# andreaskoepf/faster-rcnn.torch

Hardware: AMD Instinct MI355X
Metric: images/sec (vgg_small 800x450 fwd+bwd) (higher is better)
Workload: dtype f32 (conv / Linear(13824,1024) operands as 2 x fp16 split planes: 22 significand bits, 3 MFMA partial products; fp32 accumulate)

## Files before the change

### faster-rcnn.torch_amd/_lib.py

```python
import ctypes as C
import os

_HERE = os.path.dirname(os.path.abspath(__file__))
SO_PATH = os.environ.get("FRCNN_LIB_PATH") or os.path.join(_HERE, "libfrcnn_hip.so")

KC_NAMES = ["conv_igemm_k3", "conv_igemm_other", "conv_wgrad_k3", "conv_wgrad_other", "gemm", "elemwise",
            "roi", "rpn", "nms", "optim", "image", "conv_x3", "conv_wgradx", "soft_nms", "topk"]


class FrcnnError(RuntimeError):
    pass


class ModelDesc(C.Structure):
    _fields_ = [
        ("nblocks", C.c_int),
        ("filters", C.c_int * 8), ("ksize", C.c_int * 8), ("pad", C.c_int * 8), ("conv_steps", C.c_int * 8),
        ("dropout", C.c_float * 8),
        ("nheads", C.c_int),
        ("head_k", C.c_int * 8), ("head_n", C.c_int * 8), ("head_input", C.c_int * 8),
        ("ncls", C.c_int),
        ("cls_n", C.c_int * 8), ("cls_bn", C.c_int * 8),
        ("cls_dropout", C.c_float * 8),
        ("class_count", C.c_int),
# ... 31 lines not shown
    "frcnn_nms_device_batch": ([vp, C.c_int, C.c_longlong, C.c_int, vp, C.c_int, C.c_float, C.c_int, C.c_int, vp, vp, vp, vp, C.c_size_t,
                               vp], C.c_int),
    "frcnn_soft_nms_workspace_bytes": ([C.c_int, C.c_int], C.c_size_t),
    "frcnn_soft_nms_batch": ([vp, C.c_int, C.c_longlong, C.c_int, vp, C.c_int, C.c_int, C.c_int, C.c_float, C.c_float, C.c_float, C.c_int,
                             vp, vp, vp, vp, C.c_longlong, vp, C.c_size_t, vp], C.c_int),
    "frcnn_topk_select_workspace_bytes": ([C.c_int, C.c_int], C.c_size_t),
    "frcnn_topk_select": ([vp, C.c_int, C.c_longlong, C.c_int, vp, C.c_int, vp, C.c_longlong, vp, vp, C.c_size_t, vp], C.c_int),
    "frcnn_rpn_gather_rows": ([vp, vp, vp, vp, C.c_int, C.c_longlong, C.c_int, vp, C.c_longlong, vp, C.c_int, vp, vp, vp, vp, vp, vp,
                              C.c_longlong, vp], C.c_int),
    "frcnn_detect_gather_batch": ([vp, vp, C.c_int, C.c_int, vp, vp, vp, vp, vp, C.c_longlong, vp, vp, vp, vp, vp], C.c_int),
    "frcnn_roi_windows": ([vp, vp, C.c_int, vp, C.c_int, C.c_int, C.c_int, vp, vp], C.c_int),
    "frcnn_detect_post": ([vp, vp, vp, vp, vp, C.c_int, C.c_int, C.c_double, vp, vp, vp, vp, vp, vp], C.c_int),
    "frcnn_nms_host": ([vp, C.c_int, C.c_int, C.c_float, C.c_int, C.c_int, vp, vp], C.c_int),
    "frcnn_conv2d_forward": ([vp, C.c_int, C.c_int, C.c_int, vp, vp, vp, vp, C.c_int, C.c_int, C.c_int, vp, vp], C.c_int),
    "frcnn_conv2d_backward_input": ([vp, C.c_int, C.c_int, C.c_int, vp, C.c_int, C.c_int, C.c_int, vp, C.c_int, vp], C.c_int),
    "frcnn_conv2d_backward_weight": ([vp, C.c_int, C.c_int, C.c_int, vp, vp, vp, C.c_int, C.c_int, C.c_int, vp, vp, vp], C.c_int),
    "frcnn_maxpool_act_forward": ([vp, C.c_int, C.c_int, C.c_int, vp, vp, vp, vp, vp], C.c_int),
    "frcnn_maxpool_act_backward": ([vp, vp, vp, C.c_int, C.c_int, C.c_int, vp, vp, vp, vp, vp, vp], C.c_int),
    "frcnn_act_forward": ([vp, C.c_int, C.c_longlong, vp, vp, vp, vp], C.c_int),
    "frcnn_act_backward": ([vp, vp, C.c_int, C.c_longlong, vp, vp, vp, vp, vp, vp], C.c_int),
    "frcnn_amax_record_floats": ([], C.c_int),
    "frcnn_tensor_absmax": ([vp, C.c_longlong, vp, vp], C.c_int),
    "frcnn_maxpool_act_forward_rec": ([vp, C.c_int, C.c_int, C.c_int, vp, vp, vp, vp, vp, vp], C.c_int),
    "frcnn_maxpool_act_backward_rec": ([vp, vp, vp, C.c_int, C.c_int, C.c_int, vp, vp, vp, vp, vp, vp, vp], C.c_int),
    "frcnn_act_backward_rec": ([vp, vp, C.c_int, C.c_longlong, vp, vp, vp, vp, vp, vp, vp], C.c_int),
    "frcnn_conv2d_forward_rec": ([vp, C.c_int, C.c_int, C.c_int, vp, vp, vp, vp, C.c_int, C.c_int, C.c_int, vp, vp, vp, vp], C.c_int),
    "frcnn_conv2d_backward_input_rec": ([vp, C.c_int, C.c_int, C.c_int, vp, C.c_int, C.c_int, C.c_int, vp, C.c_int, vp, vp, vp, vp, vp, vp,
                                         vp], C.c_int),
    "frcnn_roi_pool_forward": ([vp, C.c_int, C.c_int, C.c_int, vp, C.c_int, C.c_int, C.c_int, vp, vp, vp], C.c_int),
    "frcnn_roi_pool_backward": ([vp, C.c_int, C.c_int, C.c_int, vp, vp, C.c_int, C.c_int, C.c_int, vp], C.c_int),
# ... 125 lines not shown
```

### faster-rcnn.torch_amd/csrc/api.cpp

```cpp
#include <cmath>
#include <cstring>
#include <vector>
#include <mutex>

#include "kernels.h"

namespace frcnn {

static thread_local std::string g_err;

void set_error(const char* fmt, ...) {
  char buf[1024];
  va_list ap;
  va_start(ap, fmt);
  vsnprintf(buf, sizeof(buf), fmt, ap);
  va_end(ap);
  g_err = buf;
}

struct ProfRec { int klass; double flops, bytes; hipEvent_t a, b; hipStream_t s; };
static hipEvent_t g_prof_base = nullptr;
static unsigned g_prof_mask = 0;
static std::vector<ProfRec> g_recs;
static std::vector<hipEvent_t> g_pool;
// ... 206 lines not shown
  return FRCNN_OK;
}

static int scale_fits_f16_form(const float* in_scale, int C, hipStream_t s, bool* ok) {
  *ok = true;
  if (!in_scale) return FRCNN_OK;
  std::vector<float> h((size_t)C);
  FR_HIP(hipMemcpyAsync(h.data(), in_scale, (size_t)C * 4, hipMemcpyDeviceToHost, s));
  FR_HIP(hipStreamSynchronize(s));
  for (float v : h) if (!(std::fabs(v) <= 1.f)) { *ok = false; break; }
  return FRCNN_OK;
}

static int conv2d_split(const float* in, int Kc, int H, int W, const float* in_slope, const float* in_scale, const float* weight,
                        const float* bias, int O, int C, int M, int k, int mode, int pad, float* out, int out_mode, bool f16,
                        const float* rec_in, float* rec_out, const X3PostAct* post, hipStream_t s) {
  float* wp = nullptr;
  FR_HIP(hipMalloc((void**)&wp, conv_x3_pack_bytes(Kc, M, k)));
  float* am = nullptr;
  int rcx = f16 ? x3_f16_records(&am) : FRCNN_OK;
  float* const amw = am ? am + AMAX_REC : nullptr;
  float* const aws = am ? am + 2 * AMAX_REC : nullptr;
  if (am && rcx == FRCNN_OK) {
    if (!rec_in) rcx = tensor_absmax(in, (long)Kc * H * W, am, s);
    if (rcx == FRCNN_OK) rcx = tensor_absmax(weight, (long)O * C * k * k, amw, s);
  }
  if (rcx == FRCNN_OK) rcx = conv_x3_pack(weight, O, C, k, mode, wp, s, H + 2 * pad - k + 1, W + 2 * pad - k + 1, amw, aws);
  if (rcx == FRCNN_OK)
    rcx = conv_x3(in, Kc, H, W, in_slope, in_scale, wp, bias, M, k, pad, out, out_mode, 0, s, 0, post, am ? (rec_in ? rec_in : am) : nullptr,
                  aws, rec_out);
  (void)hipStreamSynchronize(s);
  (void)hipFree(wp); (void)hipFree(am);
  return rcx;
}

int frcnn_conv2d_forward(const float* in, int C, int H, int W, const float* in_slope, const float* in_scale,
                         const float* weight, const float* bias, int O, int k, int pad, float* out,
                         void* stream) {
  float* wf = nullptr;
  if (conv_x3_eligible(C, O, k) && (k == 3 || (!in_slope && !in_scale))) {
    bool unit = true;
    FR_TRY(scale_fits_f16_form(in_scale, C, S(stream), &unit));
    return conv2d_split(in, C, H, W, in_slope, in_scale, weight, bias, O, C, O, k, 0, pad, out, OUT_STORE, unit, nullptr, nullptr, nullptr,
                        S(stream));
  }
// ... 6 lines not shown
}
int frcnn_conv2d_backward_input(const float* gout, int O, int Ho, int Wo, const float* weight, int C, int k,
                                int pad, float* gin, int accumulate, void* stream) {
  float* wd = nullptr;
  if (conv_x3_eligible(O, C, k))
    return conv2d_split(gout, O, Ho, Wo, nullptr, nullptr, weight, nullptr, O, C, C, k, 1, k - 1 - pad, gin, accumulate ? OUT_ADD : OUT_STORE,
                        true, nullptr, nullptr, nullptr, S(stream));
  FR_HIP(hipMalloc((void**)&wd, conv_pack_floats(O, C, k) * 4));
  int rc = conv_pack_weights(weight, O, C, k, nullptr, wd, S(stream));
  if (rc == FRCNN_OK)
    rc = conv_igemm(gout, O, Ho, Wo, nullptr, nullptr, wd, nullptr, C, k, k - 1 - pad, gin,
                    accumulate ? OUT_ADD : OUT_STORE, 0, S(stream));
  (void)hipStreamSynchronize(S(stream));
  (void)hipFree(wd);
  return rc;
}
int frcnn_amax_record_floats(void) { return AMAX_REC; }
int frcnn_tensor_absmax(const float* x, long long n, float* rec, void* stream) {
  FR_CHECK(x && rec && n >= 1, "frcnn_tensor_absmax: bad arguments");
  return tensor_absmax(x, (long)n, rec, S(stream));
}
int frcnn_conv2d_forward_rec(const float* in, int C, int H, int W, const float* in_slope, const float* in_scale, const float* weight,
                             const float* bias, int O, int k, int pad, float* out, const float* rec_in, float* rec_out, void* stream) {
  FR_CHECK(in && weight && out, "frcnn_conv2d_forward_rec: NULL argument");
  FR_CHECK(conv_x3_eligible(C, O, k) && (k == 3 || (!in_slope && !in_scale)),
           "frcnn_conv2d_forward_rec: %d channels -> %d filters, %dx%d does not take the split form", C, O, k, k);
  FR_CHECK(get_x3_f16(), "frcnn_conv2d_forward_rec: option x3_f16 is off");
  bool unit = true;
  FR_TRY(scale_fits_f16_form(in_scale, C, S(stream), &unit));
  FR_CHECK(unit, "frcnn_conv2d_forward_rec: an entry of in_scale exceeds 1: the launch would not take the fp16 form");
// ... 315 lines not shown
```

### faster-rcnn.torch_amd/csrc/convx.hip

```cpp
#include <cstdlib>

#include "kernels.h"
#include "amax.h"
#include <type_traits>
#ifdef CX_TRACE
#include <cstdio>
#include <vector>
#endif

namespace frcnn {

typedef float f32x16 __attribute__((ext_vector_type(16)));
typedef __bf16 bf16x8 __attribute__((ext_vector_type(8)));
typedef __bf16 bf16x2 __attribute__((ext_vector_type(2)));
typedef float f32x2 __attribute__((ext_vector_type(2)));
typedef _Float16 f16x8 __attribute__((ext_vector_type(8)));
typedef _Float16 f16x2 __attribute__((ext_vector_type(2)));

#define CX_BM 128
#define CX_CH 16
#define CX_OCC 3
#define CX_PP 204
constexpr int cx_pp(int k) { return k == 3 ? CX_PP : k == 5 ? 240 : 308; }
#define CX_NA 2
// ... 9 lines not shown
#define CX_ASTAGE (6 * CX_BM * 16)

static int g_splitbf16 = -1;
void set_split_bf16(int on) { g_splitbf16 = on ? 1 : 0; }
int get_split_bf16() {
  if (g_splitbf16 < 0) g_splitbf16 = getenv("FRCNN_SPLIT_BF16") ? (atoi(getenv("FRCNN_SPLIT_BF16")) != 0) : 1;
  return g_splitbf16;
}

static int g_x3_f16 = -1;
void set_x3_f16(int on) { g_x3_f16 = on ? 1 : 0; }
int get_x3_f16() {
  if (g_x3_f16 < 0) g_x3_f16 = getenv("FRCNN_X3_F16") ? (atoi(getenv("FRCNN_X3_F16")) != 0) : 1;
  return g_x3_f16;
}

bool conv_x3_eligible(int Cin, int M, int k) {
  return get_split_bf16() && (k == 3 || k == 5 || k == 7) && Cin % CX_CH == 0 && Cin >= CX_CH && M % (k == 3 ? 64 : 128) == 0;
}

static void x3_choose_tile(int Ho, int Wo, int k, int* TH, int* TW);
int conv_x3_bm(int M, int Ho, int Wo, int k) {
  if (M % 128 != 0) return 64;
  if (k != 3 || Ho <= 0) return 128;
  int TH, TW;
  x3_choose_tile(Ho, Wo, k, &TH, &TW);
  const long tiles = (long)cdiv(Ho, TH) * cdiv(Wo, TW);
  const long b128 = tiles * (M / 128), b64 = tiles * (M / 64);
  return (b128 < 512 && b64 >= 512 && b64 <= 256 * CX_OCC) ? 64 : 128;
}
// ... 925 lines not shown
    if (FILE* f = fopen(tfile, "w")) {
      fprintf(f, "# grid %d M %d Cin %d Ho %d Wo %d TH %d TW %d splitK %d wide %d WM %d EPI %d\n", grid, a.M, a.Cin, a.Ho, a.Wo, a.TH, a.TW, a.splitK, a.wide, WM, EPI);
      for (int b = 0; b < grid; ++b) {
        for (int j = 0; j < 64; ++j) fprintf(f, "%llu ", hst[(size_t)b * 64 + j]);
        fprintf(f, "\n");
      }
      fclose(f);
    }
  }
#endif
  return FRCNN_OK;
}

int conv_x3(const float* in, int Cin, int H, int W, const float* in_slope, const float* in_scale, const void* wp,
            const float* bias, int M, int k, int pad, float* out, int out_mode, double algo_flops, hipStream_t s, int ws_slot,
            const X3PostAct* post, const float* amax_in, const float* amax_w, float* amax_out) {
  FR_CHECK((k == 3 || k == 5 || k == 7) && Cin % CX_CH == 0 && M % 64 == 0,
           "conv_x3: %d channels -> %d filters, %dx%d is not a split-bf16 shape", Cin, M, k, k);
  FR_CHECK((double)Cin * H * W * 4.0 < 4294967295.0, "conv_x3: input tensor too large for 32-bit offsets");
  CxArgs a;
  a.in = in; a.in_slope = in_slope; a.in_scale = in_scale; a.wp = wp; a.bias = bias; a.out = out;
  a.amax_in = amax_in; a.amax_w = amax_w; a.amax_out = amax_out;
  const bool f16 = amax_in != nullptr;
  FR_CHECK(!f16 || amax_w, "conv_x3: the two-plane fp16 form needs the magnitudes of both tensors");
  a.Cin = Cin; a.H = H; a.W = W; a.M = M; a.pad = pad;
  a.Ho = H + 2 * pad - k + 1; a.Wo = W + 2 * pad - k + 1;
  FR_CHECK(a.Ho > 0 && a.Wo > 0, "conv_x3: empty output (%dx%d, k=%d, pad=%d)", H, W, k, pad);
  x3_choose_tile(a.Ho, a.Wo, k, &a.TH, &a.TW);
  a.tilesX = cdiv(a.Wo, a.TW); a.tilesY = cdiv(a.Ho, a.TH);
  const int bm = conv_x3_bm(M, a.Ho, a.Wo, k);
  a.mTiles = M / bm;
// ... 36 lines not shown
  } else if (post && a.splitK == 1) {
    rc = bm == 128 ? launch_x3<3, 2, false, false, 1>(a, algo_flops, s) : launch_x3<3, 1, false, false, 1>(a, algo_flops, s);
  } else if (k == 3 && bm == 128) {
    rc = act == 3 ? launch_x3<3, 2, true, true>(a, algo_flops, s) : act == 2 ? launch_x3<3, 2, true, false>(a, algo_flops, s)
       : act == 1 ? launch_x3<3, 2, false, true>(a, algo_flops, s) : launch_x3<3, 2, false, false>(a, algo_flops, s);
  } else if (k == 3) {
    rc = act == 3 ? launch_x3<3, 1, true, true>(a, algo_flops, s) : act == 2 ? launch_x3<3, 1, true, false>(a, algo_flops, s)
       : act == 1 ? launch_x3<3, 1, false, true>(a, algo_flops, s) : launch_x3<3, 1, false, false>(a, algo_flops, s);
  } else {
    FR_CHECK(act == 0 && bm == 128, "conv_x3: a %dx%d launch takes no fused input activation and 128-filter blocks", k, k);
    rc = k == 5 ? launch_x3<5, 2, false, false>(a, algo_flops, s) : launch_x3<7, 2, false, false>(a, algo_flops, s);
  }
  FR_TRY(rc);
  if (amax_out && !slab && (long)a.tilesX * a.tilesY * a.mTiles > AMAX_MAX_BLOCKS)
    FR_TRY(tensor_absmax(out, (long)M * a.Ho * a.Wo, amax_out, s));
  if (slab) {
    long total = (long)M * a.Ho * a.Wo;
    int grid;
    const long hw = (long)a.Ho * a.Wo;
    const X3PostAct pa = post ? *post : X3PostAct{nullptr, nullptr, nullptr, nullptr};
    const bool al = ((uintptr_t)out & 15) == 0 && ((uintptr_t)a.out & 15) == 0 && (!post || ((uintptr_t)post->x & 15) == 0);
    const int vec = al && hw % 4 == 0 ? 4 : al && hw % 2 == 0 ? 2 : 1;
    grid = (int)std::min<long>(cdivl(total / vec, 256), 4096);
    if (vec == 4)
      FR_LAUNCH(KC_ELEMWISE, 0, total * 4.0 * (a.splitK + 1), s, x3_splitk_reduce_kernel<4>, dim3(grid), dim3(256), 0,
                (const float*)a.out, a.splitK, M, hw, bias, out, out_mode == OUT_ADD ? 1 : 0, pa, amax_out);
    else if (vec == 2)
      FR_LAUNCH(KC_ELEMWISE, 0, total * 4.0 * (a.splitK + 1), s, x3_splitk_reduce_kernel<2>, dim3(grid), dim3(256), 0,
                (const float*)a.out, a.splitK, M, hw, bias, out, out_mode == OUT_ADD ? 1 : 0, pa, amax_out);
    else
// ... 9 lines not shown
```

### faster-rcnn.torch_amd/csrc/elem.hip

```cpp
#include <algorithm>

#include <mutex>
#include <unordered_map>

#include "kernels.h"
#include "amax.h"

namespace frcnn {

__device__ __forceinline__ float wave_sum(float v) {
#pragma unroll
  for (int o = 32; o > 0; o >>= 1) v += __shfl_down(v, o, 64);
  return v;
}

__device__ __forceinline__ float block_sum(float v, float* sh) {
  v = wave_sum(v);
  const int lane = threadIdx.x & 63, w = threadIdx.x >> 6;
  if (lane == 0) sh[w] = v;
  __syncthreads();
  float r = 0.f;
  if (threadIdx.x < 64) {
    r = threadIdx.x < (blockDim.x >> 6) ? sh[threadIdx.x] : 0.f;
    r = wave_sum(r);
// ... 129 lines not shown
}
int maxpool_act_forward(const float* x, int C, int H, int W, const float* slope, const float* scale,
                        float* out, unsigned char* idx, hipStream_t s, float* amax) {
  int Ho = (H - 2 + 1) / 2 + 1, Wo = (W - 2 + 1) / 2 + 1;
  long total = (long)C * Ho * Wo;
  int grid = (int)std::min<long>(std::max<long>(1, cdivl(total, 256)), 4096);
  FR_LAUNCH(KC_ELEMWISE, 0, (double)C * H * W * 4.0 + total * 5.0, s, maxpool_act_forward_kernel, dim3(grid),
            dim3(256), 0, x, C, H, W, Ho, Wo, slope, scale, out, idx, amax);
  FR_LAUNCH_CHECK();
  return FRCNN_OK;
}

#ifndef ACT_BWD_THREADS
#define ACT_BWD_THREADS 512
#endif
template <bool POOLED, bool VEC>
__global__ __launch_bounds__(ACT_BWD_THREADS) void act_backward_kernel(const float* __restrict__ gin, const unsigned char* __restrict__ idx,
                                    const float* __restrict__ x, int C, int H, int W, int Ho, int Wo,
                                    const float* slope, const float* scale, float* __restrict__ gx,
                                    float* gbias, float* gslope, int chunks, float* part_b, float* part_a, float* amax) {
  __shared__ float sh[16];
  __shared__ double shd[16];
  float am = 0.f;
  const int c = blockIdx.x / chunks, chunk = blockIdx.x % chunks;
  const long hw = (long)H * W;
  long per = cdivl(hw, chunks);
  if (VEC) per = (per + 3) & ~3L;
  const long beg = chunk * per, end = beg + per < hw ? beg + per : hw;
  const float a = slope ? *slope : 1.f;
  const float sc = scale ? scale[c] : 1.f;
  const bool has_slope = slope != nullptr;
  float sb = 0.f;
  double sa = 0.0;
  if (VEC) {
    const float* xc = x + (size_t)c * hw;
    const float* gc = POOLED ? gin + (size_t)c * Ho * Wo : gin + (size_t)c * hw;
    const unsigned char* ic = POOLED ? idx + (size_t)c * Ho * Wo : nullptr;
    float* oc = gx + (size_t)c * hw;
    const unsigned ibeg = (unsigned)beg, iend = (unsigned)end, uW = (unsigned)W, stride = 4u * blockDim.x;
    auto fetch = [&](unsigned i, bool ok, float* g, float4& xv4) {
      if (!ok) { g[0] = g[1] = g[2] = g[3] = 0.f; xv4 = make_float4(1.f, 1.f, 1.f, 1.f); return; }
      if (POOLED) {
        const unsigned y = i / uW, xx = i - y * uW;
        const unsigned po = (y >> 1) * (unsigned)Wo + (xx >> 1);
        const float2 gp = *reinterpret_cast<const float2*>(gc + po);
        const unsigned short ib = *reinterpret_cast<const unsigned short*>(ic + po);
        const unsigned char code = (unsigned char)((y & 1) * 2);
        g[0] = ((ib & 0xff) == code) ? gp.x : 0.f;
        g[1] = ((ib & 0xff) == code + 1) ? gp.x : 0.f;
        g[2] = ((ib >> 8) == code) ? gp.y : 0.f;
        g[3] = ((ib >> 8) == code + 1) ? gp.y : 0.f;
      } else {
        const float4 gv = *reinterpret_cast<const float4*>(gc + i);
        g[0] = gv.x; g[1] = gv.y; g[2] = gv.z; g[3] = gv.w;
      }
      xv4 = *reinterpret_cast<const float4*>(xc + i);
    };
    auto finish = [&](unsigned i, const float* g, const float4& xv4) {
      const float xv[4] = {xv4.x, xv4.y, xv4.z, xv4.w};
      float r[4];
// ... 13 lines not shown
      const bool ok2 = i2 < iend;
      float g0[4], g1[4];
      float4 x0, x1;
      fetch(i, true, g0, x0);
      fetch(i2, ok2, g1, x1);
      finish(i, g0, x0);
      if (ok2) finish(i2, g1, x1);
    }
  } else {
    for (long i = beg + threadIdx.x; i < end; i += blockDim.x) {
      float g;
      if (POOLED) {
        int y = (int)(i / W), xx = (int)(i - (long)y * W);
        int oy = y >> 1, ox = xx >> 1;
        long po = ((long)c * Ho + oy) * Wo + ox;
        g = (idx[po] == (unsigned char)((y & 1) * 2 + (xx & 1))) ? gin[po] : 0.f;
      } else {
        g = gin[(size_t)c * hw + i];
      }
      if (scale) g *= sc;
      float xv = x[(size_t)c * hw + i];
      float r = g;
      if (has_slope) {
        if (!(xv > 0.f)) { r = a * g; sa += (double)xv * (double)g; }
      }
      gx[(size_t)c * hw + i] = r;
      sb += r;
      am = fmaxf(am, fabsf(r));
    }
  }
  if (amax) amax_store_block(am, amax);
// ... 49 lines not shown
    FR_HIP(hipMalloc((void**)&e.first, n * 4));
    e.second = n;
  }
  *out = e.first;
  return FRCNN_OK;
}

static int act_bwd_chunks(int C, long hw) {
  long want = cdivl(512, C);
  long maxc = cdivl(hw, 4096);
  return (int)std::max<long>(1, std::min<long>(want, maxc));
}

int maxpool_act_backward(const float* gpool, const unsigned char* idx, const float* x, int C, int H,
                         int W, const float* slope, const float* scale, float* gx, float* gbias,
                         float* gslope, hipStream_t s, float* amax) {
  int Ho = (H - 2 + 1) / 2 + 1, Wo = (W - 2 + 1) / 2 + 1;
  int chunks = act_bwd_chunks(C, (long)H * W);
  float* const amax_after = (amax && (long)C * chunks > AMAX_MAX_BLOCKS) ? amax : nullptr;
  if (amax_after) amax = nullptr;
  float *pb = nullptr, *pa = nullptr;
  if (deterministic()) { FR_TRY(det_workspace(s, (size_t)2 * C * chunks, &pb)); pa = pb + (size_t)C * chunks; }
  const bool vec = (W % 4 == 0) && (Wo % 2 == 0) && (((uintptr_t)gpool | (uintptr_t)x | (uintptr_t)gx) % 16 == 0) &&
                   ((uintptr_t)idx % 2 == 0);
  if (vec)
    FR_LAUNCH(KC_ELEMWISE, 0, (double)C * H * W * 9.25, s, (act_backward_kernel<true, true>), dim3(C * chunks),
              dim3(ACT_BWD_THREADS), 0, gpool, idx, x, C, H, W, Ho, Wo, slope, scale, gx, gbias, gslope, chunks, pb, pa, amax);
  else
    FR_LAUNCH(KC_ELEMWISE, 0, (double)C * H * W * 9.25, s, (act_backward_kernel<true, false>), dim3(C * chunks),
              dim3(ACT_BWD_THREADS), 0, gpool, idx, x, C, H, W, Ho, Wo, slope, scale, gx, gbias, gslope, chunks, pb, pa, amax);
  FR_LAUNCH_CHECK();
  if (pb) FR_TRY(fold_partials(gbias ? pb : nullptr, (slope && gslope) ? pa : nullptr, C, chunks, gbias, gslope, s));
  if (amax_after) FR_TRY(tensor_absmax(gx, (long)C * H * W, amax_after, s));
  return FRCNN_OK;
}

int act_backward(const float* gy, const float* x, int C, long hw, const float* slope,
                 const float* scale, float* gx, float* gbias, float* gslope, hipStream_t s, float* amax) {
  int chunks = act_bwd_chunks(C, hw);
  float* const amax_after = (amax && (long)C * chunks > AMAX_MAX_BLOCKS) ? amax : nullptr;
  if (amax_after) amax = nullptr;
  float *pb = nullptr, *pa = nullptr;
  if (deterministic()) { FR_TRY(det_workspace(s, (size_t)2 * C * chunks, &pb)); pa = pb + (size_t)C * chunks; }
  const bool vec = (hw % 4 == 0) && (((uintptr_t)gy | (uintptr_t)x | (uintptr_t)gx) % 16 == 0);
  if (vec)
    FR_LAUNCH(KC_ELEMWISE, 0, (double)C * hw * 12.0, s, (act_backward_kernel<false, true>), dim3(C * chunks),
              dim3(ACT_BWD_THREADS), 0, gy, (const unsigned char*)nullptr, x, C, 1, (int)hw, 1, 1, slope, scale, gx,
              gbias, gslope, chunks, pb, pa, amax);
  else
    FR_LAUNCH(KC_ELEMWISE, 0, (double)C * hw * 12.0, s, (act_backward_kernel<false, false>), dim3(C * chunks),
              dim3(ACT_BWD_THREADS), 0, gy, (const unsigned char*)nullptr, x, C, 1, (int)hw, 1, 1, slope, scale, gx,
              gbias, gslope, chunks, pb, pa, amax);
  FR_LAUNCH_CHECK();
  if (pb) FR_TRY(fold_partials(gbias ? pb : nullptr, (slope && gslope) ? pa : nullptr, C, chunks, gbias, gslope, s));
  if (amax_after) FR_TRY(tensor_absmax(gx, (long)C * hw, amax_after, s));
  return FRCNN_OK;
}

__global__ void channel_sum_kernel(const float* __restrict__ g, long hw, float* gbias, int chunks, float* part_b) {
  __shared__ float sh[16];
  const int c = blockIdx.x / chunks, chunk = blockIdx.x % chunks;
  long per = cdivl(hw, chunks);
  per = (per + 3) & ~3L;
  const long beg = chunk * per, end = beg + per < hw ? beg + per : hw;
  const float* gc = g + (size_t)c * hw;
  float sb = 0.f;
  if (beg < end) {
// ... 588 lines not shown
```

### faster-rcnn.torch_amd/csrc/kernels.h

```cpp
#pragma once
#include <algorithm>

#include "common.h"

namespace frcnn {

int conv_cc(int k);
int conv_mpad(int M);
size_t conv_pack_floats(int Kchan, int M, int k);
int conv_pack_weights(const float* w, int O, int C, int k, float* wf, float* wd, hipStream_t s);
struct PackJob { long w_off; long total; float* dst; int O, C, k, mode, Mpad, blk_begin, nblk; };
PackJob conv_pack_job(long w_off, int O, int C, int k, int mode, float* dst);
int conv_pack_assign_blocks(PackJob* jobs, int njobs, int total_blocks);
int conv_pack_weights_multi(const float* weights, const PackJob* jobs_dev, int njobs, int grid, hipStream_t s);

enum { OUT_STORE = 0, OUT_ADD = 1 };
struct IgemmPool { float* out; unsigned char* idx; const float* slope; const float* scale; float* amax = nullptr; };
int conv_igemm(const float* in, int Cin, int H, int W, const float* in_slope, const float* in_scale,
               const float* wp, const float* bias, int M, int k, int pad, float* out, int out_mode,
               double algo_flops, hipStream_t s, int ws_slot = 0,
               const IgemmPool* pool = nullptr, bool* pool_fused = nullptr);

void set_split_bf16(int on);
int get_split_bf16();
// ... 5 lines not shown
};
PackXJob conv_x3_pack_job(long w_off, int O, int C, int k, int mode, void* dst, int Ho, int Wo);
int conv_x3_pack_assign_blocks(PackXJob* jobs, int njobs);
int conv_x3_pack_multi(const float* weights, const PackXJob* jobs_dev, int njobs, int grid, hipStream_t s);
int conv_x3_pack(const float* w, int O, int C, int k, int mode, void* dst, hipStream_t s, int Ho, int Wo,
                 const float* amax_rec_w = nullptr, float* amax_w = nullptr);
#define AMAX_REC 16400
#define AMAX_MAX_BLOCKS 16384
int tensor_absmax(const float* x, long n, float* rec, hipStream_t s);
struct AmaxJob { long off; long n; float* out; int blk_begin; };
int tensor_absmax_assign_blocks(AmaxJob* jobs, int njobs);
long tensor_absmax_record_floats(long n);
int tensor_absmax_multi(const float* w, const AmaxJob* jobs_dev, int njobs, int grid, hipStream_t s);
void set_x3_f16(int on);
int get_x3_f16();
int conv_x3(const float* in, int Cin, int H, int W, const float* in_slope, const float* in_scale, const void* wp,
            const float* bias, int M, int k, int pad, float* out, int out_mode, double algo_flops, hipStream_t s, int ws_slot = 0,
            const struct X3PostAct* post = nullptr, const float* amax_in = nullptr, const float* amax_w = nullptr,
            float* amax_out = nullptr);
struct X3PostAct {
  const float* x;
  const float* slope;
  const float* scale;
  float* gslope;
};

bool conv_wgradx_eligible(int Cin, int O, int k);
size_t conv_wgradx_workspace_bytes(int Cin, int H, int W, int O, int pad);
struct WgradMap { const int* omap = nullptr; const int* cmap = nullptr; int Cfull = 0; };
int conv_wgradx(const float* in, int Cin, int H, int W, const float* in_slope, const float* in_scale, const float* g, int O,
                int pad, float* gw, void* ws, size_t ws_bytes, hipStream_t s, float* gbias = nullptr,
                const float* amax_in = nullptr, const float* amax_g = nullptr,
                const WgradMap* map = nullptr);
int wgrad_reduce(const float* slab, int nSplit, int taps, int OC, float* gw, hipStream_t s);
// ... 11 lines not shown
               const WgradMap* map = nullptr);

bool deterministic();
void set_deterministic(bool on);
int det_workspace(hipStream_t s, size_t floats, float** out);

int fill_zero(void* p, size_t bytes, hipStream_t s);
int scale_inplace(float* x, long n, float sc, hipStream_t s);
int add_inplace(float* y, const float* x, long n, hipStream_t s);
int act_forward(const float* x, int C, long hw, const float* slope, const float* scale, float* y,
                hipStream_t s);
int maxpool_act_forward(const float* x, int C, int H, int W, const float* slope, const float* scale,
                        float* out, unsigned char* idx, hipStream_t s, float* amax = nullptr);
int maxpool_act_backward(const float* gpool, const unsigned char* idx, const float* x, int C, int H,
                         int W, const float* slope, const float* scale, float* gx, float* gbias,
                         float* gslope, hipStream_t s, float* amax = nullptr);
int act_backward(const float* gy, const float* x, int C, long hw, const float* slope,
                 const float* scale, float* gx, float* gbias, float* gslope, hipStream_t s, float* amax = nullptr);
int channel_sum(const float* g, int C, long hw, float* gbias, hipStream_t s);
int channel_sum_cols(const float* g, int R, int O, float* gb, hipStream_t s);
int gather_positions(const float* src, int C, long hw, const int* pos, int P, float* dst, const float* slope,
                     float* dst_act, hipStream_t s);
int im2col_positions(const float* X, int C, int H, int W, int k, int Wo, const int* pos, int P, float* col, hipStream_t s);
int col2im_positions_add(const float* col, int C, int H, int W, int k, int Wo, const int* pos, int P, float* gX,
                         hipStream_t s);
int dropout_channel_mask(float* scale, int C, float p, unsigned long long seed, hipStream_t s);
int fill_value(float* x, long n, float v, hipStream_t s);
int rmsprop_step(float* x, float* g, float* m, long n, float lr, float alpha, float eps, float gscale,
                 bool scale_first, hipStream_t s, const double* gcount_dev = nullptr);
int rmsprop_slice(float* x, float* g, float* m, long lo, long hi, float lr, float alpha, float eps, float gscale, bool scale_first,
                  hipStream_t s, const double* gcount_dev = nullptr);
// ... 173 lines not shown
```

### faster-rcnn.torch_amd/csrc/net.cpp

```cpp
#include <array>
#include <vector>
#include <cmath>
#include <cstring>

#include "kernels.h"

namespace frcnn {

static const int HEAD_OUT = 18;
static const int SPARSE_MAX_POS = 512;

struct DevBuf {
  void* p = nullptr;
  size_t bytes = 0;
  bool owned = true;
  void view(void* ptr, size_t n) { p = ptr; bytes = n; owned = false; }
  int ensure(size_t need) {
    if (need <= bytes) return FRCNN_OK;
    if (p && owned) (void)hipFree(p);
    owned = true;
    p = nullptr; bytes = 0;
    FR_HIP(hipMalloc(&p, need + 64));
    bytes = need;
    return FRCNN_OK;
// ... 664 lines not shown
  return FRCNN_OK;
}

int frcnn_get_option(const char* name, int* value) {
  FR_CHECK(name != nullptr && value != nullptr, "get_option: null argument");
  if (strcmp(name, "side_stream") == 0) { *value = side_enabled() ? 1 : 0; return FRCNN_OK; }
  if (strcmp(name, "gemm_x_roles") == 0) { *value = get_gemm_x_roles(); return FRCNN_OK; }
  if (strcmp(name, "deterministic") == 0) { *value = deterministic() ? 1 : 0; return FRCNN_OK; }
  if (strcmp(name, "static_weights") == 0) { *value = g_static_weights; return FRCNN_OK; }
  if (strcmp(name, "drop_compact") == 0) { *value = drop_compact_on(); return FRCNN_OK; }
  if (strcmp(name, "sparse_heads") == 0) { *value = sparse_heads_on(); return FRCNN_OK; }
  if (strcmp(name, "winograd") == 0) { *value = 0; return FRCNN_OK; }
  if (strcmp(name, "cnet_wgrad_async") == 0) { *value = g_cnet_wgrad_async; return FRCNN_OK; }
  if (strcmp(name, "split_bf16") == 0) { *value = get_split_bf16(); return FRCNN_OK; }
  if (strcmp(name, "x3_f16") == 0) { *value = get_x3_f16(); return FRCNN_OK; }
  FR_CHECK(false, "get_option: unknown option '%s'", name);
  return FRCNN_OK;
}

int frcnn_set_option(const char* name, int value) {
  FR_CHECK(name != nullptr, "set_option: null name");
  if (strcmp(name, "side_stream") == 0) { g_side_stream = value ? 1 : 0; return FRCNN_OK; }
  if (strcmp(name, "deterministic") == 0) { set_deterministic(value != 0); return FRCNN_OK; }
  if (strcmp(name, "static_weights") == 0) { g_static_weights = value != 0; ++g_static_gen; return FRCNN_OK; }
  if (strcmp(name, "drop_compact") == 0) { g_drop_compact = value != 0; return FRCNN_OK; }
  if (strcmp(name, "sparse_heads") == 0) { g_sparse_heads = value != 0; return FRCNN_OK; }
  if (strcmp(name, "gemm_x_roles") == 0) { set_gemm_x_roles(value); return FRCNN_OK; }
  if (strcmp(name, "split_bf16") == 0) { set_split_bf16(value); return FRCNN_OK; }
  if (strcmp(name, "x3_f16") == 0) { set_x3_f16(value); return FRCNN_OK; }
  if (strcmp(name, "winograd") == 0) return FRCNN_OK;
  if (strcmp(name, "cnet_wgrad_async") == 0) { g_cnet_wgrad_async = value ? 1 : 0; return FRCNN_OK; }
  FR_CHECK(false, "set_option: unknown option '%s'", name);
  return FRCNN_OK;
}

static int ensure_head_streams(frcnn_model* m);
static int ensure_side(frcnn_model* m) {
  if (!m->side) {
    FR_TRY(pool_stream(0, &m->side));
    FR_HIP(hipEventCreateWithFlags(&m->join_ev, hipEventDisableTiming));
    FR_HIP(hipEventCreateWithFlags(&m->loss_ev, hipEventDisableTiming));
    FR_HIP(hipEventCreateWithFlags(&m->chain_ev, hipEventDisableTiming));
    for (auto& h : m->heads) FR_HIP(hipEventCreateWithFlags(&h.done, hipEventDisableTiming));
  }
// ... 845 lines not shown
  for (int b = 0; b < fb; ++b) {
    while (m->block_ev.size() < (size_t)nb) {
      hipEvent_t e;
      FR_HIP(hipEventCreateWithFlags(&e, hipEventDisableTiming));
      m->block_ev.push_back(e);
    }
    FR_HIP(hipEventRecord(m->block_ev[b], s));
    FR_TRY(record_block_read(m, b, s));
  }
  const bool use_side = side_enabled();
  if (use_side) FR_TRY(ensure_side(m));
  hipStream_t ws = use_side ? m->side : s;
  size_t n_fork = 0;
  const bool fuse_act = !deterministic() && !(getenv("FRCNN_FUSE_ACT") && atoi(getenv("FRCNN_FUSE_ACT")) == 0);
  bool act_done = false;
  for (int b = nb - 1; b >= fb; --b) {
    Block& blk = m->blocks[b];
    for (int st = blk.nconv - 1; st >= 0; --st) {
      Conv& c = m->convs[blk.first_conv + st];
      const float* scale = (st == 0 && blk.has_drop) ? blk.scale.f() : nullptr;
      const bool fused_here = act_done;
      act_done = false;
      static const bool first_pooled_on = !(getenv("FRCNN_FIRST_POOLED") && atoi(getenv("FRCNN_FIRST_POOLED")) == 0);
      const bool first_pooled = fuse_act && first_pooled_on && b == 0 && st == 0 && blk.nconv == 1 && scale == nullptr &&
                                conv_wgrad_first_pooled_eligible(c.Cin, c.Cout, c.k, c.Wo);
      if (first_pooled) {
        FR_TRY(conv_wgrad_first_pooled(m->img.f(), c.Cin, c.H, c.W, blk.gpooled.f(), (const unsigned char*)blk.pidx.p, c.x.f(),
                                       w + c.a_off, c.Cout, c.pad, grad + c.w_off, grad + c.b_off, grad + c.a_off,
                                       m->wg_ws_first.p, m->wg_ws_first.bytes, s));
        while (m->block_ev.size() < (size_t)nb) {
          hipEvent_t e;
          FR_HIP(hipEventCreateWithFlags(&e, hipEventDisableTiming));
          m->block_ev.push_back(e);
        }
        FR_HIP(hipEventRecord(m->block_ev[b], s));
        FR_TRY(record_block_read(m, b, s));
        break;
      }
      if (fused_here) {
      } else if (st == blk.nconv - 1) {
        FR_TRY(maxpool_act_backward(blk.gpooled.f(), (const unsigned char*)blk.pidx.p, c.x.f(), c.Cout, c.Ho, c.Wo,
                                    w + c.a_off, scale, c.gx.f(), grad + c.b_off, grad + c.a_off, s,
                                    (c.x_d && m->f16_packed) ? m->rec_w(c.am + 1) : nullptr));
      } else {
        FR_TRY(act_backward(c.gx.f(), c.x.f(), c.Cout, (long)c.Ho * c.Wo, w + c.a_off, scale, c.gx.f(),
                            grad + c.b_off, grad + c.a_off, s, (c.x_d && m->f16_packed) ? m->rec_w(c.am + 1) : nullptr));
      }
      const float* in; const float* in_slope = nullptr; const float* in_scale = nullptr;
      if (st > 0) {
        Conv& pc = m->convs[blk.first_conv + st - 1];
        in = pc.x.f(); in_slope = w + pc.a_off;
        in_scale = (st - 1 == 0 && blk.has_drop) ? blk.scale.f() : nullptr;
      } else {
        in = b == 0 ? m->img.f() : m->blocks[b - 1].pooled.f();
      }
      const bool dc = blk.dc_on && st <= 1;
      int wg_cin = c.Cin, wg_o = c.Cout;
      WgradMap wmap;
// ... 31 lines not shown
        break;
      }
      float* gin = st > 0 ? m->convs[blk.first_conv + st - 1].gx.f() : m->blocks[b - 1].gpooled.f();
      const int gmode = st > 0 ? OUT_STORE : OUT_ADD;
      const float* ag = nullptr;
      const float* aw = nullptr;
      if (c.x_d && m->f16_packed) { ag = m->rec(c.am + 1); aw = m->amax_ws.f() + c.am; }
      const int dg_k = (dc && st == 0) ? blk.nkK : c.Cout, dg_m = (dc && st == 1) ? blk.nkM : c.Cin;
      const double fl = 2.0 * dg_k * dg_m * c.k * c.k * (double)c.Ho * c.Wo;
      if (c.x_d && st > 0 && fuse_act && c.k == 3) {
        Conv& pc = m->convs[blk.first_conv + st - 1];
        X3PostAct post{pc.x.f(), w + pc.a_off, (st - 1 == 0 && blk.has_drop && !dc) ? blk.scale.f() : nullptr, grad + pc.a_off};
        FR_TRY(conv_x3(c.gx.f(), dg_k, c.Ho, c.Wo, nullptr, nullptr, c.wxd.p, nullptr, dg_m, c.k, c.k - 1 - c.pad, gin, gmode, fl, s, 0, &post, ag, aw,
                       (pc.x_d && m->f16_packed) ? m->rec_w(pc.am + 1) : nullptr));
        act_done = true;
      } else if (c.x_d)
        FR_TRY(conv_x3(c.gx.f(), dg_k, c.Ho, c.Wo, nullptr, nullptr, c.wxd.p, nullptr, dg_m, c.k, c.k - 1 - c.pad, gin, gmode, fl, s, 0, nullptr, ag, aw));
      else
        FR_TRY(conv_igemm(c.gx.f(), c.Cout, c.Ho, c.Wo, nullptr, nullptr, c.wd.f(), nullptr, c.Cin, c.k,
                          c.k - 1 - c.pad, gin, gmode, fl, s));
      if (st == 0) FR_TRY(record_block_read(m, b, s));
    }
  }
  m->block_ev_valid = true;
  if (heads_tail && !m->heads_gin) FR_TRY(join_heads(m, s));
  FR_TRY(cw_join(m, s));
  if (use_side) {
    FR_HIP(hipEventRecord(m->join_ev, ws));
    FR_HIP(hipStreamWaitEvent(s, m->join_ev, 0));
    m->side_busy = false;
  }
  return FRCNN_OK;
}
// ... 242 lines not shown
```

### include/frcnn_hip.h

```cpp
#ifndef FRCNN_HIP_H
#define FRCNN_HIP_H

#include <stddef.h>

#ifdef __cplusplus
extern "C" {
#endif

#define FRCNN_OK 0
#define FRCNN_ERR_ARG 1
#define FRCNN_ERR_HIP 2
#define FRCNN_ERR_STATE 3

int frcnn_version(void);
const char *frcnn_last_error(void);
int frcnn_device_count(int *n);
int frcnn_set_device(int device);
int frcnn_device_name(char *buf_host, int len);
int frcnn_set_option(const char *name, int value);
int frcnn_get_option(const char *name, int *value_host);

int frcnn_malloc(void **ptr_out_host, size_t bytes);
int frcnn_free(void *ptr);
int frcnn_host_alloc(void **ptr_out_host, size_t bytes);
// ... 47 lines not shown
int frcnn_roi_windows(const double *rect, const long long *pick, int k, const int *layers_host, int nlayers, int fmH, int fmW,
                      int *wins, void *stream);
int frcnn_detect_post(const int *cls, const float *conf, const float *bbox, const double *rect, const long long *pick, int R,
                      int bgclass, double min_conf, float *bb, int *kc, int *keep_row, double *r2, int *K_dev, void *stream);
int frcnn_detect_gather_batch(const long long *wpick, const int *counts, int B, int row_stride, const int *keep_row,
                              const int *kc, const float *bb, const double *r2, const long long *pick, long long match_stride,
                              const float *match_p, const double *match_rect, const int *match_idx, double *rec, void *stream);
int frcnn_nms_host(const float *boxes_host, int n, int ncols, float overlap, int key_mode,
                   int key_col, long long *pick_host, int *count_host);

int frcnn_conv2d_forward(const float *in, int C, int H, int W, const float *in_slope,
                         const float *in_scale, const float *weight, const float *bias, int O,
                         int k, int pad, float *out, void *stream);
int frcnn_conv2d_backward_input(const float *gout, int O, int Ho, int Wo, const float *weight,
                                int C, int k, int pad, float *gin, int accumulate, void *stream);
int frcnn_conv2d_backward_weight(const float *in, int C, int H, int W, const float *in_slope,
                                 const float *in_scale, const float *gout, int O, int k, int pad,
                                 float *gweight, float *gbias, void *stream);

int frcnn_maxpool_act_forward(const float *x, int C, int H, int W, const float *slope,
                              const float *scale, float *out, unsigned char *idx, void *stream);
int frcnn_maxpool_act_backward(const float *gpool, const unsigned char *idx, const float *x, int C,
                               int H, int W, const float *slope, const float *scale, float *gx,
                               float *gbias, float *gslope, void *stream);
int frcnn_act_forward(const float *x, int C, long long hw, const float *slope, const float *scale,
                      float *y, void *stream);
int frcnn_act_backward(const float *gy, const float *x, int C, long long hw, const float *slope,
                       const float *scale, float *gx, float *gbias, float *gslope, void *stream);

int frcnn_amax_record_floats(void);
// ... 200 lines not shown
```

Measured before the change: 518.7.

## Defer split-K slab reduction of dgrad conv into pooled activation backward

When the split-K backward-input convolution writes into the previous block's pooled gradient, the slab reduction is skipped and handed to the following maxpool/activation backward kernel. That kernel then sums the split-K partial slabs (plus the existing value in add mode) inline, removing one reduction pass and one write and read of the pooled gradient. A new API entry and an option toggle are added. The risk is extra strided slab reads inside the elementwise kernel and reliance on the slab staying valid until the consumer runs.

```diff
diff --git a/faster-rcnn.torch_amd/_lib.py b/faster-rcnn.torch_amd/_lib.py
--- a/faster-rcnn.torch_amd/_lib.py
+++ b/faster-rcnn.torch_amd/_lib.py
@@ -69,6 +69,8 @@
     "frcnn_nms_host": ([vp, C.c_int, C.c_int, C.c_float, C.c_int, C.c_int, vp, vp], C.c_int),
     "frcnn_conv2d_forward": ([vp, C.c_int, C.c_int, C.c_int, vp, vp, vp, vp, C.c_int, C.c_int, C.c_int, vp, vp], C.c_int),
     "frcnn_conv2d_backward_input": ([vp, C.c_int, C.c_int, C.c_int, vp, C.c_int, C.c_int, C.c_int, vp, C.c_int, vp], C.c_int),
+    "frcnn_conv2d_backward_input_pool": ([vp, C.c_int, C.c_int, C.c_int, vp, C.c_int, C.c_int, C.c_int, vp, C.c_int, vp, vp, C.c_int, C.c_int,
+                                          vp, vp, vp, vp, vp, vp, vp], C.c_int),
     "frcnn_conv2d_backward_weight": ([vp, C.c_int, C.c_int, C.c_int, vp, vp, vp, C.c_int, C.c_int, C.c_int, vp, vp, vp], C.c_int),
     "frcnn_maxpool_act_forward": ([vp, C.c_int, C.c_int, C.c_int, vp, vp, vp, vp, vp], C.c_int),
     "frcnn_maxpool_act_backward": ([vp, vp, vp, C.c_int, C.c_int, C.c_int, vp, vp, vp, vp, vp, vp], C.c_int),
diff --git a/faster-rcnn.torch_amd/csrc/api.cpp b/faster-rcnn.torch_amd/csrc/api.cpp
--- a/faster-rcnn.torch_amd/csrc/api.cpp
+++ b/faster-rcnn.torch_amd/csrc/api.cpp
@@ -244,7 +244,7 @@
 
 static int conv2d_split(const float* in, int Kc, int H, int W, const float* in_slope, const float* in_scale, const float* weight,
                         const float* bias, int O, int C, int M, int k, int mode, int pad, float* out, int out_mode, bool f16,
-                        const float* rec_in, float* rec_out, const X3PostAct* post, hipStream_t s) {
+                        const float* rec_in, float* rec_out, const X3PostAct* post, hipStream_t s, X3Fold* defer = nullptr) {
   float* wp = nullptr;
   FR_HIP(hipMalloc((void**)&wp, conv_x3_pack_bytes(Kc, M, k)));
   float* am = nullptr;
@@ -258,7 +258,7 @@
   if (rcx == FRCNN_OK) rcx = conv_x3_pack(weight, O, C, k, mode, wp, s, H + 2 * pad - k + 1, W + 2 * pad - k + 1, amw, aws);
   if (rcx == FRCNN_OK)
     rcx = conv_x3(in, Kc, H, W, in_slope, in_scale, wp, bias, M, k, pad, out, out_mode, 0, s, 0, post, am ? (rec_in ? rec_in : am) : nullptr,
-                  aws, rec_out);
+                  aws, rec_out, defer);
   (void)hipStreamSynchronize(s);
   (void)hipFree(wp); (void)hipFree(am);
   return rcx;
@@ -295,6 +295,21 @@
   (void)hipStreamSynchronize(S(stream));
   (void)hipFree(wd);
   return rc;
+}
+int frcnn_conv2d_backward_input_pool(const float* gout, int O, int Ho, int Wo, const float* weight, int C, int k, int pad, float* gin,
+                                     int accumulate, const unsigned char* idx, const float* x, int xH, int xW, const float* slope,
+                                     const float* scale, float* gx, float* gbias, float* gslope, float* rec, void* stream) {
+  FR_CHECK(gout && weight && gin && idx && x && gx, "frcnn_conv2d_backward_input_pool: NULL argument");
+  const int Hi = Ho + k - 1 - 2 * pad, Wi = Wo + k - 1 - 2 * pad;
+  FR_CHECK(xH >= 1 && xW >= 1 && (xH - 1) / 2 + 1 == Hi && (xW - 1) / 2 + 1 == Wi,
+           "frcnn_conv2d_backward_input_pool: x of %d x %d does not pool to the %d x %d map the convolution reads", xH, xW, Hi, Wi);
+  X3Fold fold;
+  if (conv_x3_eligible(O, C, k))
+    FR_TRY(conv2d_split(gout, O, Ho, Wo, nullptr, nullptr, weight, nullptr, O, C, C, k, 1, k - 1 - pad, gin, accumulate ? OUT_ADD : OUT_STORE,
+                        true, nullptr, nullptr, nullptr, S(stream), x3_consumer_fold_on() ? &fold : nullptr));
+  else
+    FR_TRY(frcnn_conv2d_backward_input(gout, O, Ho, Wo, weight, C, k, pad, gin, accumulate, stream));
+  return maxpool_act_backward(gin, idx, x, C, xH, xW, slope, scale, gx, gbias, gslope, S(stream), rec, &fold);
 }
 int frcnn_amax_record_floats(void) { return AMAX_REC; }
 int frcnn_tensor_absmax(const float* x, long long n, float* rec, void* stream) {
diff --git a/faster-rcnn.torch_amd/csrc/convx.hip b/faster-rcnn.torch_amd/csrc/convx.hip
--- a/faster-rcnn.torch_amd/csrc/convx.hip
+++ b/faster-rcnn.torch_amd/csrc/convx.hip
@@ -47,6 +47,10 @@
   if (g_x3_f16 < 0) g_x3_f16 = getenv("FRCNN_X3_F16") ? (atoi(getenv("FRCNN_X3_F16")) != 0) : 1;
   return g_x3_f16;
 }
+static int g_x3_consumer_fold = 1;
+void set_x3_consumer_fold(int on) { g_x3_consumer_fold = on ? 1 : 0; }
+int get_x3_consumer_fold() { return g_x3_consumer_fold; }
+bool x3_consumer_fold_on() { return g_x3_consumer_fold != 0 && !deterministic(); }
 
 bool conv_x3_eligible(int Cin, int M, int k) {
   return get_split_bf16() && (k == 3 || k == 5 || k == 7) && Cin % CX_CH == 0 && Cin >= CX_CH && M % (k == 3 ? 64 : 128) == 0;
@@ -1002,7 +1006,8 @@
 
 int conv_x3(const float* in, int Cin, int H, int W, const float* in_slope, const float* in_scale, const void* wp,
             const float* bias, int M, int k, int pad, float* out, int out_mode, double algo_flops, hipStream_t s, int ws_slot,
-            const X3PostAct* post, const float* amax_in, const float* amax_w, float* amax_out) {
+            const X3PostAct* post, const float* amax_in, const float* amax_w, float* amax_out, X3Fold* defer) {
+  if (defer) *defer = X3Fold{};
   FR_CHECK((k == 3 || k == 5 || k == 7) && Cin % CX_CH == 0 && M % 64 == 0,
            "conv_x3: %d channels -> %d filters, %dx%d is not a split-bf16 shape", Cin, M, k, k);
   FR_CHECK((double)Cin * H * W * 4.0 < 4294967295.0, "conv_x3: input tensor too large for 32-bit offsets");
@@ -1069,6 +1074,10 @@
   FR_TRY(rc);
   if (amax_out && !slab && (long)a.tilesX * a.tilesY * a.mTiles > AMAX_MAX_BLOCKS)
     FR_TRY(tensor_absmax(out, (long)M * a.Ho * a.Wo, amax_out, s));
+  if (slab && defer && !post && !bias && !amax_out && (out_mode == OUT_ADD || out_mode == OUT_STORE)) {
+    defer->slab = (const float*)a.out; defer->nSplit = a.splitK; defer->total = (long)M * a.Ho * a.Wo; defer->add = out_mode == OUT_ADD;
+    return FRCNN_OK;
+  }
   if (slab) {
     long total = (long)M * a.Ho * a.Wo;
     int grid;
diff --git a/faster-rcnn.torch_amd/csrc/elem.hip b/faster-rcnn.torch_amd/csrc/elem.hip
--- a/faster-rcnn.torch_amd/csrc/elem.hip
+++ b/faster-rcnn.torch_amd/csrc/elem.hip
@@ -167,11 +167,13 @@
 #ifndef ACT_BWD_THREADS
 #define ACT_BWD_THREADS 512
 #endif
-template <bool POOLED, bool VEC>
+template <bool POOLED, bool VEC, int FOLD = 0>
 __global__ __launch_bounds__(ACT_BWD_THREADS) void act_backward_kernel(const float* __restrict__ gin, const unsigned char* __restrict__ idx,
                                     const float* __restrict__ x, int C, int H, int W, int Ho, int Wo,
                                     const float* slope, const float* scale, float* __restrict__ gx,
-                                    float* gbias, float* gslope, int chunks, float* part_b, float* part_a, float* amax) {
+                                    float* gbias, float* gslope, int chunks, float* part_b, float* part_a, float* amax,
+                                    X3Fold fold = X3Fold{}) {
+  static_assert(POOLED || !FOLD, "only the pooled form folds");
   __shared__ float sh[16];
   __shared__ double shd[16];
   float am = 0.f;
@@ -196,7 +198,37 @@
       if (POOLED) {
         const unsigned y = i / uW, xx = i - y * uW;
         const unsigned po = (y >> 1) * (unsigned)Wo + (xx >> 1);
-        const float2 gp = *reinterpret_cast<const float2*>(gc + po);
+        float2 gp;
+        if (FOLD) {
+          const float* fp = fold.slab + (size_t)c * Ho * Wo + po;
+          const size_t T = (size_t)fold.total;
+          const float2 o = *reinterpret_cast<const float2*>(gc + po);
+          gp = make_float2(0.f, 0.f);
+          if (FOLD >= 2) {
+            float2 t[FOLD >= 2 ? FOLD : 1];
+#pragma unroll
+            for (int j = 0; j < FOLD; ++j) t[j] = *reinterpret_cast<const float2*>(fp + (size_t)j * T);
+#pragma unroll
+            for (int j = 0; j < FOLD; ++j) { gp.x += t[j].x; gp.y += t[j].y; }
+          } else {
+            int sp = 0;
+            for (; sp + 4 <= fold.nSplit; sp += 4) {
+              float2 t[4];
+#pragma unroll
+              for (int j = 0; j < 4; ++j) t[j] = *reinterpret_cast<const float2*>(fp + (size_t)(sp + j) * T);
+#pragma unroll
+              for (int j = 0; j < 4; ++j) { gp.x += t[j].x; gp.y += t[j].y; }
+            }
+            for (; sp < fold.nSplit; ++sp) {
+              const float2 t0 = *reinterpret_cast<const float2*>(fp + (size_t)sp * T);
+              gp.x += t0.x; gp.y += t0.y;
+            }
+          }
+          gp.x += fold.add ? o.x : 0.f;
+          gp.y += fold.add ? o.y : 0.f;
+        } else {
+          gp = *reinterpret_cast<const float2*>(gc + po);
+        }
         const unsigned short ib = *reinterpret_cast<const unsigned short*>(ic + po);
         const unsigned char code = (unsigned char)((y & 1) * 2);
         g[0] = ((ib & 0xff) == code) ? gp.x : 0.f;
@@ -240,7 +272,13 @@
         int y = (int)(i / W), xx = (int)(i - (long)y * W);
         int oy = y >> 1, ox = xx >> 1;
         long po = ((long)c * Ho + oy) * Wo + ox;
-        g = (idx[po] == (unsigned char)((y & 1) * 2 + (xx & 1))) ? gin[po] : 0.f;
+        if (FOLD) {
+          float v = 0.f;
+          for (int sp = 0; sp < fold.nSplit; ++sp) v += fold.slab[(size_t)sp * (size_t)fold.total + po];
+          if (fold.add) v += gin[po];
+          g = (idx[po] == (unsigned char)((y & 1) * 2 + (xx & 1))) ? v : 0.f;
+        } else
+          g = (idx[po] == (unsigned char)((y & 1) * 2 + (xx & 1))) ? gin[po] : 0.f;
       } else {
         g = gin[(size_t)c * hw + i];
       }
@@ -320,21 +358,35 @@
 
 int maxpool_act_backward(const float* gpool, const unsigned char* idx, const float* x, int C, int H,
                          int W, const float* slope, const float* scale, float* gx, float* gbias,
-                         float* gslope, hipStream_t s, float* amax) {
+                         float* gslope, hipStream_t s, float* amax, const X3Fold* fold) {
   int Ho = (H - 2 + 1) / 2 + 1, Wo = (W - 2 + 1) / 2 + 1;
   int chunks = act_bwd_chunks(C, (long)H * W);
+  const bool folds = fold && fold->nSplit > 0;
+  FR_CHECK(!folds || (fold->slab && gpool && fold->total == (long)C * Ho * Wo),
+           "maxpool_act_backward: the deferred fold covers %ld values, the pooled map %ld", folds ? fold->total : 0L, (long)C * Ho * Wo);
   float* const amax_after = (amax && (long)C * chunks > AMAX_MAX_BLOCKS) ? amax : nullptr;
   if (amax_after) amax = nullptr;
   float *pb = nullptr, *pa = nullptr;
   if (deterministic()) { FR_TRY(det_workspace(s, (size_t)2 * C * chunks, &pb)); pa = pb + (size_t)C * chunks; }
   const bool vec = (W % 4 == 0) && (Wo % 2 == 0) && (((uintptr_t)gpool | (uintptr_t)x | (uintptr_t)gx) % 16 == 0) &&
                    ((uintptr_t)idx % 2 == 0);
-  if (vec)
+  if (folds) {
+    const double bytes = (double)C * H * W * 8.25 + (double)fold->total * 4.0 * (fold->nSplit + (fold->add ? 1 : 0));
+#define ACT_BWD_FOLD(VEC_, N_)                                                                                                      \
+  FR_LAUNCH(KC_ELEMWISE, 0, bytes, s, (act_backward_kernel<true, VEC_, N_>), dim3(C * chunks), dim3(ACT_BWD_THREADS), 0, gpool, idx, \
+            x, C, H, W, Ho, Wo, slope, scale, gx, gbias, gslope, chunks, pb, pa, amax, *fold)
+    if (!(vec && (uintptr_t)fold->slab % 16 == 0)) ACT_BWD_FOLD(false, 1);
+    else if (fold->nSplit == 2) ACT_BWD_FOLD(true, 2);
+    else if (fold->nSplit == 3) ACT_BWD_FOLD(true, 3);
+    else if (fold->nSplit == 4) ACT_BWD_FOLD(true, 4);
+    else ACT_BWD_FOLD(true, 1);
+#undef ACT_BWD_FOLD
+  } else if (vec)
     FR_LAUNCH(KC_ELEMWISE, 0, (double)C * H * W * 9.25, s, (act_backward_kernel<true, true>), dim3(C * chunks),
-              dim3(ACT_BWD_THREADS), 0, gpool, idx, x, C, H, W, Ho, Wo, slope, scale, gx, gbias, gslope, chunks, pb, pa, amax);
+              dim3(ACT_BWD_THREADS), 0, gpool, idx, x, C, H, W, Ho, Wo, slope, scale, gx, gbias, gslope, chunks, pb, pa, amax, X3Fold{});
   else
     FR_LAUNCH(KC_ELEMWISE, 0, (double)C * H * W * 9.25, s, (act_backward_kernel<true, false>), dim3(C * chunks),
-              dim3(ACT_BWD_THREADS), 0, gpool, idx, x, C, H, W, Ho, Wo, slope, scale, gx, gbias, gslope, chunks, pb, pa, amax);
+              dim3(ACT_BWD_THREADS), 0, gpool, idx, x, C, H, W, Ho, Wo, slope, scale, gx, gbias, gslope, chunks, pb, pa, amax, X3Fold{});
   FR_LAUNCH_CHECK();
   if (pb) FR_TRY(fold_partials(gbias ? pb : nullptr, (slope && gslope) ? pa : nullptr, C, chunks, gbias, gslope, s));
   if (amax_after) FR_TRY(tensor_absmax(gx, (long)C * H * W, amax_after, s));
@@ -352,11 +404,11 @@
   if (vec)
     FR_LAUNCH(KC_ELEMWISE, 0, (double)C * hw * 12.0, s, (act_backward_kernel<false, true>), dim3(C * chunks),
               dim3(ACT_BWD_THREADS), 0, gy, (const unsigned char*)nullptr, x, C, 1, (int)hw, 1, 1, slope, scale, gx,
-              gbias, gslope, chunks, pb, pa, amax);
+              gbias, gslope, chunks, pb, pa, amax, X3Fold{});
   else
     FR_LAUNCH(KC_ELEMWISE, 0, (double)C * hw * 12.0, s, (act_backward_kernel<false, false>), dim3(C * chunks),
               dim3(ACT_BWD_THREADS), 0, gy, (const unsigned char*)nullptr, x, C, 1, (int)hw, 1, 1, slope, scale, gx,
-              gbias, gslope, chunks, pb, pa, amax);
+              gbias, gslope, chunks, pb, pa, amax, X3Fold{});
   FR_LAUNCH_CHECK();
   if (pb) FR_TRY(fold_partials(gbias ? pb : nullptr, (slope && gslope) ? pa : nullptr, C, chunks, gbias, gslope, s));
   if (amax_after) FR_TRY(tensor_absmax(gx, (long)C * hw, amax_after, s));
diff --git a/faster-rcnn.torch_amd/csrc/kernels.h b/faster-rcnn.torch_amd/csrc/kernels.h
--- a/faster-rcnn.torch_amd/csrc/kernels.h
+++ b/faster-rcnn.torch_amd/csrc/kernels.h
@@ -43,10 +43,15 @@
 int tensor_absmax_multi(const float* w, const AmaxJob* jobs_dev, int njobs, int grid, hipStream_t s);
 void set_x3_f16(int on);
 int get_x3_f16();
+struct X3Fold { const float* slab = nullptr; int nSplit = 0; long total = 0; bool add = false; };
+void set_x3_consumer_fold(int on);
+int get_x3_consumer_fold();
+bool x3_consumer_fold_on();
 int conv_x3(const float* in, int Cin, int H, int W, const float* in_slope, const float* in_scale, const void* wp,
             const float* bias, int M, int k, int pad, float* out, int out_mode, double algo_flops, hipStream_t s, int ws_slot = 0,
             const struct X3PostAct* post = nullptr, const float* amax_in = nullptr, const float* amax_w = nullptr,
-            float* amax_out = nullptr);
+            float* amax_out = nullptr,
+            X3Fold* defer = nullptr);
 struct X3PostAct {
   const float* x;
   const float* slope;
@@ -88,7 +93,8 @@
                         float* out, unsigned char* idx, hipStream_t s, float* amax = nullptr);
 int maxpool_act_backward(const float* gpool, const unsigned char* idx, const float* x, int C, int H,
                          int W, const float* slope, const float* scale, float* gx, float* gbias,
-                         float* gslope, hipStream_t s, float* amax = nullptr);
+                         float* gslope, hipStream_t s, float* amax = nullptr,
+                         const X3Fold* fold = nullptr);
 int act_backward(const float* gy, const float* x, int C, long hw, const float* slope,
                  const float* scale, float* gx, float* gbias, float* gslope, hipStream_t s, float* amax = nullptr);
 int channel_sum(const float* g, int C, long hw, float* gbias, hipStream_t s);
diff --git a/faster-rcnn.torch_amd/csrc/net.cpp b/faster-rcnn.torch_amd/csrc/net.cpp
--- a/faster-rcnn.torch_amd/csrc/net.cpp
+++ b/faster-rcnn.torch_amd/csrc/net.cpp
@@ -702,6 +702,7 @@
   if (strcmp(name, "cnet_wgrad_async") == 0) { *value = g_cnet_wgrad_async; return FRCNN_OK; }
   if (strcmp(name, "split_bf16") == 0) { *value = get_split_bf16(); return FRCNN_OK; }
   if (strcmp(name, "x3_f16") == 0) { *value = get_x3_f16(); return FRCNN_OK; }
+  if (strcmp(name, "x3_consumer_fold") == 0) { *value = get_x3_consumer_fold(); return FRCNN_OK; }
   FR_CHECK(false, "get_option: unknown option '%s'", name);
   return FRCNN_OK;
 }
@@ -716,6 +717,7 @@
   if (strcmp(name, "gemm_x_roles") == 0) { set_gemm_x_roles(value); return FRCNN_OK; }
   if (strcmp(name, "split_bf16") == 0) { set_split_bf16(value); return FRCNN_OK; }
   if (strcmp(name, "x3_f16") == 0) { set_x3_f16(value); return FRCNN_OK; }
+  if (strcmp(name, "x3_consumer_fold") == 0) { set_x3_consumer_fold(value); return FRCNN_OK; }
   if (strcmp(name, "winograd") == 0) return FRCNN_OK;
   if (strcmp(name, "cnet_wgrad_async") == 0) { g_cnet_wgrad_async = value ? 1 : 0; return FRCNN_OK; }
   FR_CHECK(false, "set_option: unknown option '%s'", name);
@@ -1591,6 +1593,13 @@
   size_t n_fork = 0;
   const bool fuse_act = !deterministic() && !(getenv("FRCNN_FUSE_ACT") && atoi(getenv("FRCNN_FUSE_ACT")) == 0);
   bool act_done = false;
+  static const bool first_pooled_on = !(getenv("FRCNN_FIRST_POOLED") && atoi(getenv("FRCNN_FIRST_POOLED")) == 0);
+  auto first_pooled_block = [&](int b) {
+    const Block& k = m->blocks[b];
+    const Conv& c0 = m->convs[k.first_conv];
+    return fuse_act && first_pooled_on && b == 0 && k.nconv == 1 && !k.has_drop && conv_wgrad_first_pooled_eligible(c0.Cin, c0.Cout, c0.k, c0.Wo);
+  };
+  X3Fold carried;
   for (int b = nb - 1; b >= fb; --b) {
     Block& blk = m->blocks[b];
     for (int st = blk.nconv - 1; st >= 0; --st) {
@@ -1598,9 +1607,7 @@
       const float* scale = (st == 0 && blk.has_drop) ? blk.scale.f() : nullptr;
       const bool fused_here = act_done;
       act_done = false;
-      static const bool first_pooled_on = !(getenv("FRCNN_FIRST_POOLED") && atoi(getenv("FRCNN_FIRST_POOLED")) == 0);
-      const bool first_pooled = fuse_act && first_pooled_on && b == 0 && st == 0 && blk.nconv == 1 && scale == nullptr &&
-                                conv_wgrad_first_pooled_eligible(c.Cin, c.Cout, c.k, c.Wo);
+      const bool first_pooled = st == 0 && first_pooled_block(b);
       if (first_pooled) {
         FR_TRY(conv_wgrad_first_pooled(m->img.f(), c.Cin, c.H, c.W, blk.gpooled.f(), (const unsigned char*)blk.pidx.p, c.x.f(),
                                        w + c.a_off, c.Cout, c.pad, grad + c.w_off, grad + c.b_off, grad + c.a_off,
@@ -1618,7 +1625,8 @@
       } else if (st == blk.nconv - 1) {
         FR_TRY(maxpool_act_backward(blk.gpooled.f(), (const unsigned char*)blk.pidx.p, c.x.f(), c.Cout, c.Ho, c.Wo,
                                     w + c.a_off, scale, c.gx.f(), grad + c.b_off, grad + c.a_off, s,
-                                    (c.x_d && m->f16_packed) ? m->rec_w(c.am + 1) : nullptr));
+                                    (c.x_d && m->f16_packed) ? m->rec_w(c.am + 1) : nullptr, &carried));
+        carried = X3Fold{};
       } else {
         FR_TRY(act_backward(c.gx.f(), c.x.f(), c.Cout, (long)c.Ho * c.Wo, w + c.a_off, scale, c.gx.f(),
                             grad + c.b_off, grad + c.a_off, s, (c.x_d && m->f16_packed) ? m->rec_w(c.am + 1) : nullptr));
@@ -1680,9 +1688,11 @@
         FR_TRY(conv_x3(c.gx.f(), dg_k, c.Ho, c.Wo, nullptr, nullptr, c.wxd.p, nullptr, dg_m, c.k, c.k - 1 - c.pad, gin, gmode, fl, s, 0, &post, ag, aw,
                        (pc.x_d && m->f16_packed) ? m->rec_w(pc.am + 1) : nullptr));
         act_done = true;
-      } else if (c.x_d)
-        FR_TRY(conv_x3(c.gx.f(), dg_k, c.Ho, c.Wo, nullptr, nullptr, c.wxd.p, nullptr, dg_m, c.k, c.k - 1 - c.pad, gin, gmode, fl, s, 0, nullptr, ag, aw));
-      else
+      } else if (c.x_d) {
+        X3Fold* defer = (st == 0 && b > 0 && gin == m->blocks[b - 1].gpooled.f() && x3_consumer_fold_on() && !first_pooled_block(b - 1)) ? &carried : nullptr;
+        FR_TRY(conv_x3(c.gx.f(), dg_k, c.Ho, c.Wo, nullptr, nullptr, c.wxd.p, nullptr, dg_m, c.k, c.k - 1 - c.pad, gin, gmode, fl, s, 0, nullptr, ag, aw,
+                       nullptr, defer));
+      } else
         FR_TRY(conv_igemm(c.gx.f(), c.Cout, c.Ho, c.Wo, nullptr, nullptr, c.wd.f(), nullptr, c.Cin, c.k,
                           c.k - 1 - c.pad, gin, gmode, fl, s));
       if (st == 0) FR_TRY(record_block_read(m, b, s));
diff --git a/include/frcnn_hip.h b/include/frcnn_hip.h
--- a/include/frcnn_hip.h
+++ b/include/frcnn_hip.h
@@ -85,6 +85,11 @@
                          int k, int pad, float *out, void *stream);
 int frcnn_conv2d_backward_input(const float *gout, int O, int Ho, int Wo, const float *weight,
                                 int C, int k, int pad, float *gin, int accumulate, void *stream);
+int frcnn_conv2d_backward_input_pool(const float *gout, int O, int Ho, int Wo, const float *weight,
+                                     int C, int k, int pad, float *gin, int accumulate,
+                                     const unsigned char *idx, const float *x, int xH, int xW,
+                                     const float *slope, const float *scale, float *gx, float *gbias,
+                                     float *gslope, float *rec, void *stream);
 int frcnn_conv2d_backward_weight(const float *in, int C, int H, int W, const float *in_slope,
                                  const float *in_scale, const float *gout, int O, int k, int pad,
                                  float *gweight, float *gbias, void *stream);
```

Result: no change. 526.1, median of 6 (+1.4%).
